# AIML-IfI/openset-imagenet

Measured on AMD Instinct MI355X. Metric: images/sec (whole node) ResNet-50 + entropic-open-set, Protocol 2, 1/2/4/8 GPUs, higher is better.
Workload: dtype f32; 1 GPU; Protocol 2, ResNet-50, entropic open-set loss, batch 128/GPU; workload_key=p2, classes=30, batch_per_gpu=128, global_batch=128, image=3x224x224, loss=entropic, optimizer=adam lr=1e-3, parallelism=dp1

## Files before the change

openset-imagenet_amd/csrc/conv_igemm.hip:

```cpp
#include "conv_common.h"
#include <algorithm>
#include <type_traits>

using namespace osi_conv;

namespace {

constexpr int BK = 32;
constexpr int LDR = BK + 4;

struct ConvP {
    const float* x;
    const float* w;
    float* y;
    int B, H, W, Cin, Ho, Wo, Cout, R, S, stride, pad;
    int M;
    int Ktot;
    int MT, NT;
    int accumulate;
    int x_bytes, w_bytes;
    FastDiv dHoWo, dWo;
    FastDiv cHW[4], cW[4];
    int unit;
    float* pmean;
// ... 826 lines not shown
#pragma unroll
        for (int i = 0; i < BRN; ++i) *reinterpret_cast<f32x4*>(sB + (bk_row + BRP * i) * LDC + bk_col) = rbv[i];
    };

    if (T > t0) {
        gload(); advance();
        sstore(0);
        __syncthreads();
        OSI_STAMP(p, sidx, 1);
            for (int t = t0; t < T; ++t) {
            const int buf = NST == 2 ? ((t - t0) & 1) : 0;
                if (!(OSI_ABLATE & 1)) if (t + 1 < T) { gload(); advance(); }
            const float* sA = smem + buf * STAGE;
            if (OSI_ABLATE & 16) {
#pragma unroll
                for (int j = 0; j < 16; ++j)
#pragma unroll
                    for (int i = 0; i < WM; ++i)
#pragma unroll
                        for (int n = 0; n < WN; ++n) acc[i][n] = __builtin_amdgcn_mfma_f32_32x32x2f32(ra[i % AR][j & 3], rbv[n % BRN][j & 3], acc[i][n], 0, 0, 0);
            } else if constexpr (W3) {
                const int h4 = (lane >> 5) * 4;
                const float* pa = sA + (prow + 2 - cjs) * LDR + h4;
                const float* pb = sA + AROWS * LDR + h4 * LDC + wn * 32 + (lane & 31);
#pragma unroll
                for (int j = 0; j < 4; ++j) {
                    const f32x4 a = *reinterpret_cast<const f32x4*>(pa + 8 * j);
#pragma unroll
                    for (int e = 0; e < 4; ++e) acc[0][0] = __builtin_amdgcn_mfma_f32_32x32x2f32(a[e], pb[(8 * j + e) * LDC], acc[0][0], 0, 0, 0);
                }
                if (++cjs == 3) cjs = 0;
            } else
            mma_RC<WM, WN, LDC>(sA, sA + BM * LDR, wm * 32 * WM, wn * 32 * WN, lane, acc);
            if (!(OSI_ABLATE & 4)) if (NST == 1) __syncthreads();
            if (!(OSI_ABLATE & 2)) if (t + 1 < T) sstore(NST == 2 ? (buf ^ 1) : 0);
            if (!(OSI_ABLATE & 4)) __syncthreads();
        }
        OSI_STAMP(p, sidx, 2);
    }
    if (OSI_ABLATE & 32) { if (acc[0][0][0] == 123.456f) p.y[tid] = acc[0][0][1]; return; }

    if constexpr (WM == 1 && WN == 1) {
        static_assert(BM * LDT <= STAGE, "transposed tile must fit the operand stage");
        float* tile = smem;
        tile64_to_lds<W3>(tile, acc[0][0], wm, wn, lane, m0, Mc);
        __syncthreads();
        if (KS && ks >= 0) {
            tile64_to_slab(p, tile, mt, nt, ks);
            OSI_STAMP(p, sidx, 3);
            return;
        }
        dgrad_epilogue64<FUSED, POOL>(p, smem, cls, mt, m0, n0, Mc, st, ph, pw, dHW, dW,
                                [&](int rl, int c4) { return *reinterpret_cast<const f32x4*>(tile + rl * LDT + c4 * 4); });
        OSI_STAMP(p, sidx, 3);
        return;
    }

    float esg[WN], es0[WN], es1[WN];
#pragma unroll
    for (int n = 0; n < WN; ++n) { esg[n] = 0.f; es0[n] = 0.f; es1[n] = 0.f; }
#pragma unroll
    for (int i = 0; i < WM; ++i) {
#pragma unroll
        for (int q = 0; q < 4; ++q) {
            uint32_t roff[4];
            bool rok[4];
#pragma unroll
            for (int e = 0; e < 4; ++e) {
                int m = m0 + wm * 32 * WM + i * 32 + acc_row(4 * q + e, lane);
                rok[e] = m < Mc;
                uint32_t mm = rok[e] ? (uint32_t)m : 0u;
                uint32_t pix;
                if (st == 1) pix = mm;
                else {
                    uint32_t b = fdiv(mm, dHW);
                    uint32_t rem = mm - b * dHW.d;
                    uint32_t h2 = fdiv(rem, dW), w2 = rem - h2 * dW.d;
                    pix = (b * p.H + (ph + st * h2)) * p.W + (pw + st * w2);
                }
                roff[e] = pix * p.Cin;
            }
#pragma unroll
            for (int n = 0; n < WN; ++n) {
                const int col = n0 + wn * 32 * WN + n * 32 + (lane & 31);
                float v[4];
#pragma unroll
                for (int e = 0; e < 4; ++e) v[e] = acc[i][n][4 * q + e];
                if (p.addend) {
#pragma unroll
                    for (int e = 0; e < 4; ++e) v[e] += rok[e] ? p.addend[roff[e] + col] : 0.f;
                }
                if (FUSED) {
                    if (p.ebits) {
#pragma unroll
                        for (int e = 0; e < 4; ++e) {
                            const uint32_t i4 = (roff[e] + col) >> 2;
                            const unsigned long long w = rok[e] ? p.ebits[(size_t)(i4 >> 6) * 4 + (col & 3)] : 0ull;
                            v[e] = (w >> (i4 & 63)) & 1 ? v[e] : 0.f;
                        }
                    }
                    if (p.escale0) {
                        const float gsc = p.escale0[col], gsh = p.eshift0[col];
#pragma unroll
                        for (int e = 0; e < 4; ++e)
                            v[e] = (rok[e] && __builtin_fmaf(p.ey0[roff[e] + col], gsc, gsh) > 0.f) ? v[e] : 0.f;
                    }
                    if (p.esum) {
                        const float mu0 = p.emean0[col], is0 = p.einv0[col];
#pragma unroll
                        for (int e = 0; e < 4; ++e) {
                            const float gv = rok[e] ? v[e] : 0.f;
                            esg[n] += gv;
                            es0[n] += gv * ((rok[e] ? p.ey0[roff[e] + col] : mu0) - mu0) * is0;
                        }
                        if (p.ey1) {
                            const float mu1 = p.emean1[col], is1 = p.einv1[col];
#pragma unroll
                            for (int e = 0; e < 4; ++e)
                                es1[n] += (rok[e] ? v[e] : 0.f) * ((rok[e] ? p.ey1[roff[e] + col] : mu1) - mu1) * is1;
                        }
                    }
                }
#pragma unroll
                for (int e = 0; e < 4; ++e)
                    if (rok[e]) p.y[roff[e] + col] = v[e];
            }
        }
    }
    if (FUSED && p.esum) {
#pragma unroll
        for (int n = 0; n < WN; ++n) {
            esg[n] += __shfl_xor(esg[n], 32, 64); es0[n] += __shfl_xor(es0[n], 32, 64); es1[n] += __shfl_xor(es1[n], 32, 64);
        }
        __syncthreads();
#pragma unroll
        for (int n = 0; n < WN; ++n)
            if (lane < 32) {
                float* dst = smem + (wm * BN + wn * 32 * WN + n * 32 + lane) * 3;
                dst[0] = esg[n]; dst[1] = es0[n]; dst[2] = es1[n];
            }
        __syncthreads();
        if (tid < BN) {
            const float* a = smem + tid * 3;
            const float* b = smem + (BN + tid) * 3;
            const size_t prow = (size_t)(cls * p.MT + mt) * p.Cin + n0 + tid;
            const size_t pstride = (size_t)p.eP * p.Cin;
            p.esum[prow] = a[0] + b[0];
            p.esum[pstride + prow] = a[1] + b[1];
            if (p.ey1) p.esum[2 * pstride + prow] = a[2] + b[2];
        }
    }
}

template <int WM, int WN, bool STEM, int NST, bool XF = false>
__global__ __launch_bounds__(256, NST == 1 ? (WM * WN == 4 ? 4 : (WM * WN == 2 ? 5 : 8)) : 2) void k_conv_wgrad(ConvP p) {
    static_assert(!(XF && STEM), "the stem reads the image, not an activation");
    constexpr int BM = 64 * WM, BN = 64 * WN;
    constexpr int LDA = BM + 4, LDB = BN + 4;
    constexpr int AV = BM / 4, ARP = 256 / AV, ARN = BK / ARP;
    constexpr int BV = BN / 4, BRP = 256 / BV, BRN = BK / BRP;
    constexpr int STAGE = BK * (LDA + LDB);
    extern __shared__ __attribute__((aligned(16))) float smem[];

    const int tid = threadIdx.x, lane = tid & 63, wave = tid >> 6;
    const int wm = wave >> 1, wn = wave & 1;
#ifdef OSI_STAMPS
    const size_t sidx = (size_t)blockIdx.y * gridDim.x + blockIdx.x;
#endif
    OSI_STAMP(p, sidx, 0); OSI_STAMP_ID(p, sidx);
    int mt, ntile, split;
    if (p.wgroup) {
        const int taps = STEM ? 1 : p.R * p.S;
        const int ctiles = p.NT / taps;
        const int xcd = blockIdx.x & 7, slot = blockIdx.x >> 3;
        const int u = slot % p.ginner;
        const int key = (slot / p.ginner) * 8 + xcd;
        if (key >= p.gkeys) return;
        const int tp = u % taps, v = u / taps;
        int ct;
        if (p.gkind == 0) { split = key; mt = v % p.MT; ct = v / p.MT; }
        else if (p.gkind == 1) { split = key / p.MT; mt = key - split * p.MT; ct = v; }
        else if (p.gkind == 2) { split = key / ctiles; ct = key - split * ctiles; mt = v; }
        else { mt = key % p.MT; const int rest = key / p.MT; ct = rest % ctiles; split = rest / ctiles; }
        ntile = tp * ctiles + ct;
    } else {
        mt = blockIdx.x % p.MT; ntile = blockIdx.x / p.MT; split = blockIdx.y;
    }
    const int n0 = mt * BM;
    int tap = 0, c0 = 0, r = 0, s = 0;
    if (!STEM) {
        const int ctiles = p.Cin / BN;
        tap = ntile / ctiles; c0 = (ntile - tap * ctiles) * BN;
        r = tap / p.S; s = tap - r * p.S;
    }
    const int kbeg = split * p.kchunk;
    const int kend = min(p.M, kbeg + p.kchunk);
    const int T = kend > kbeg ? (kend - kbeg + BK - 1) / BK : 0;

    f32x16 acc[WM][WN];
#pragma unroll
    for (int i = 0; i < WM; ++i)
#pragma unroll
        for (int n = 0; n < WN; ++n)
#pragma unroll
            for (int rr = 0; rr < 16; ++rr) acc[i][n][rr] = 0.f;

    const int a_row = tid / AV, a_col = (tid % AV) * 4;
    const int b_row = tid / BV, b_col = (tid % BV) * 4;
    f32x4 ra[ARN], rbv[BRN];

    const __amdgpu_buffer_rsrc_t rx = make_rsrc(p.x, p.x_bytes), rdy = make_rsrc(p.w, p.w_bytes);
    constexpr int TW = 32;
    uint32_t* tbl = reinterpret_cast<uint32_t*>(smem + NST * STAGE);
    const bool use_tbl = !STEM && p.wtbl;
    float* s_sc = smem + NST * STAGE + TW * BK;
    float* s_sh = s_sc + BN;
    if (XF) {
        if (tid < BN / 4) {
            *reinterpret_cast<f32x4*>(s_sc + tid * 4) = ld4(p.in_scale + c0 + tid * 4);
            *reinterpret_cast<f32x4*>(s_sh + tid * 4) = ld4(p.in_shift + c0 + tid * 4);
        }
        __syncthreads();
    }
    int ld_t = 0;
    auto build_tbl = [&](int t0) {
        for (int i = tid; i < TW * BK; i += 256) {
            const int m = kbeg + t0 * BK + i;
            uint32_t off = OOB;
            if (m < kend) {
                uint32_t b = fdiv((uint32_t)m, p.dHoWo);
                uint32_t rem = (uint32_t)m - b * p.dHoWo.d;
                uint32_t ho = fdiv(rem, p.dWo);
                uint32_t wo = rem - ho * p.dWo.d;
                int hi = (int)ho * p.stride - p.pad + r, wi = (int)wo * p.stride - p.pad + s;
                if ((unsigned)hi < (unsigned)p.H && (unsigned)wi < (unsigned)p.W)
                    off = (uint32_t)((((int)b * p.H + hi) * p.W + wi) * p.Cin * 4);
            }
            tbl[i] = off;
        }
        __syncthreads();
    };
    auto gload = [&](int t) {
        const int kb = kbeg + t * BK;
        ld_t = t;
#pragma unroll
        for (int i = 0; i < ARN; ++i) {
            const int m = kb + a_row + ARP * i;
            ra[i] = bld4(rdy, m < kend ? (uint32_t)(((a_row + ARP * i) * p.Cout + n0 + a_col) * 4) : OOB, (uint32_t)kb * p.Cout * 4);
        }
        if (!STEM) {
            uint32_t toff[BRN];
#pragma unroll
            for (int i = 0; i < BRN; ++i) toff[i] = tbl[(t % TW) * BK + b_row + BRP * i];
#pragma unroll
            for (int i = 0; i < BRN; ++i) {
                const int m = kb + b_row + BRP * i;
                const uint32_t uoff = m < kend ? (uint32_t)m * (uint32_t)(p.Cin * 4) : OOB;
                rbv[i] = bld4(rx, (p.unit ? uoff : toff[i]) + (uint32_t)((c0 + b_col) * 4), 0);
            }
        } else {
#pragma unroll
            for (int i = 0; i < BRN; ++i) {
                const int m = kb + b_row + BRP * i;
                bool ok = m < kend;
                uint32_t mm = ok ? (uint32_t)m : 0u;
                uint32_t b = fdiv(mm, p.dHoWo);
                uint32_t rem = mm - b * p.dHoWo.d;
                uint32_t ho = fdiv(rem, p.dWo);
                uint32_t wo = rem - ho * p.dWo.d;
                int rr = r, ss = s, coff = c0 + b_col;
                if (STEM) {
                    int tp = ntile * (BN / 4) + (b_col >> 2);
                    rr = tp / 7; ss = tp - rr * 7; coff = 0;
                    ok = ok && tp < 49;
                }
                int hi = (int)ho * p.stride - p.pad + rr, wi = (int)wo * p.stride - p.pad + ss;
                ok = ok && (unsigned)hi < (unsigned)p.H && (unsigned)wi < (unsigned)p.W;
                rbv[i] = bld4(rx, ok ? (uint32_t)(((((int)b * p.H + hi) * p.W + wi) * p.Cin + coff) * 4) : OOB, 0);
            }
        }
    };
    auto xform = [&]() {
        const f32x4 sc = *reinterpret_cast<const f32x4*>(s_sc + b_col), sh = *reinterpret_cast<const f32x4*>(s_sh + b_col);
#pragma unroll
        for (int i = 0; i < BRN; ++i) {
#pragma unroll
            for (int e = 0; e < 4; ++e) rbv[i][e] = osi_relu(__builtin_fmaf(rbv[i][e], sc[e], sh[e]));
        }
        if (!p.unit) {
#pragma unroll
            for (int i = 0; i < BRN; ++i) {
                const bool ok = tbl[(ld_t % TW) * BK + b_row + BRP * i] != OOB;
                rbv[i] = ok ? rbv[i] : f32x4{0.f, 0.f, 0.f, 0.f};
            }
        }
    };

    auto sstore = [&](int buf) {
        float* sA = smem + buf * STAGE;
        float* sB = sA + BK * LDA;
        if (XF) xform();
#pragma unroll
        for (int i = 0; i < ARN; ++i) *reinterpret_cast<f32x4*>(sA + (a_row + ARP * i) * LDA + a_col) = ra[i];
#pragma unroll
        for (int i = 0; i < BRN; ++i) *reinterpret_cast<f32x4*>(sB + (b_row + BRP * i) * LDB + b_col) = rbv[i];
    };
    if (T > 0) {
        if (use_tbl) build_tbl(0);
        gload(0);
        sstore(0);
        __syncthreads();
        OSI_STAMP(p, sidx, 1);
        for (int t = 0; t < T; ++t) {
            const int buf = NST == 2 ? (t & 1) : 0;
            if (use_tbl && t + 1 < T && (t + 1) % TW == 0) build_tbl(t + 1);
            if (!(OSI_ABLATE & 1)) if (t + 1 < T) gload(t + 1);
            const float* sA = smem + buf * STAGE;
            if (OSI_ABLATE & 16) {
#pragma unroll
                for (int ks = 0; ks < BK / 2; ++ks)
#pragma unroll
                    for (int i = 0; i < WM; ++i)
#pragma unroll
                        for (int n = 0; n < WN; ++n) acc[i][n] = __builtin_amdgcn_mfma_f32_32x32x2f32(ra[0][i & 3], rbv[0][n & 3], acc[i][n], 0, 0, 0);
            } else
            mma_CC<WM, WN, LDA, LDB>(sA, sA + BK * LDA, wm * 32 * WM, wn * 32 * WN, lane, acc);
            if (!(OSI_ABLATE & 4)) if (NST == 1) __syncthreads();
            if (!(OSI_ABLATE & 2)) if (t + 1 < T) sstore(NST == 2 ? (buf ^ 1) : 0);
            if (!(OSI_ABLATE & 4)) __syncthreads();
        }
        OSI_STAMP(p, sidx, 2);
    }

    float* out = p.y + (size_t)split * p.slab_stride;
    const int colbase = STEM ? ntile * BN : tap * p.Cin + c0;
#pragma unroll
    for (int i = 0; i < WM; ++i)
#pragma unroll
        for (int rr = 0; rr < 16; ++rr) {
            const int row = n0 + wm * 32 * WM + (WM == 2 ? 2 * acc_row(rr, lane) + i : acc_row(rr, lane));
            if constexpr (WN == 2) {
                const int col = colbase + wn * 64 + 2 * (lane & 31);
                if (col < p.Ktot) *reinterpret_cast<f32x2*>(out + (size_t)row * p.Ktot + col) = f32x2{acc[i][0][rr], acc[i][1][rr]};
            } else {
                const int col = colbase + wn * 32 + (lane & 31);
                if (col < p.Ktot) out[(size_t)row * p.Ktot + col] = acc[i][0][rr];
            }
        }
    OSI_STAMP(p, sidx, 3);
}

constexpr int W3_BKP = 32;
constexpr int W3_LDA = 64 + 16;
constexpr int W3_LDB = 32 + 16;
template <int NWIN, bool XF, bool S2 = false>
__global__ __launch_bounds__(256, 3) void k_conv_wgrad3(ConvP p) {
    extern __shared__ __attribute__((aligned(16))) float smem[];
    const int tid = threadIdx.x, lane = tid & 63, wave = tid >> 6;
    const int wn2 = wave >> 1, wc = wave & 1;
    OSI_STAMP(p, blockIdx.x, 0); OSI_STAMP_ID(p, blockIdx.x);
    const int W = p.W, WIN = S2 ? 130 + 2 * p.Wo : W3_BKP + 2 * W + 2;
    float* sA = smem;
    float* sB = sA + W3_BKP * W3_LDA;
    uint32_t* sM = reinterpret_cast<uint32_t*>(sB + NWIN * 32 * W3_LDB);
    const int ctiles = p.Cin / 32;
    int mt, ct, split;
    {
        const int xcd = blockIdx.x & 7, slot = blockIdx.x >> 3;
        const int u = slot % p.ginner, key = (slot / p.ginner) * 8 + xcd;
        if (key >= p.gkeys) return;
        if (p.gkind == 0) { split = key; mt = u % p.MT; ct = u / p.MT; }
        else { mt = key % p.MT; const int rest = key / p.MT; ct = rest % ctiles; split = rest / ctiles; }
    }
    const int n0 = mt * 64, c0 = ct * 32;
    const int kbeg = split * p.kchunk, kend = min(p.M, kbeg + p.kchunk);
    const int T = kend > kbeg ? (kend - kbeg + W3_BKP - 1) / W3_BKP : 0;

    f32x4acc acc[9][2];
#pragma unroll
    for (int t = 0; t < 9; ++t)
#pragma unroll
        for (int i = 0; i < 2; ++i) acc[t][i] = f32x4acc{0.f, 0.f, 0.f, 0.f};

    const __amdgpu_buffer_rsrc_t rx = make_rsrc(p.x, p.x_bytes), rdy = make_rsrc(p.w, p.w_bytes);
    const int a_row = tid >> 4, a_c4 = tid & 15;
    const int b_row = tid >> 3, b_c4 = tid & 7;
    f32x4 ra[2], rb[NWIN];
    f32x4 xsc = {0, 0, 0, 0}, xsh = xsc;
    if (XF) { xsc = ld4(p.in_scale + c0 + b_c4 * 4); xsh = ld4(p.in_shift + c0 + b_c4 * 4); }
    int s2_off[NWIN], s2_pq[NWIN], s2_c[NWIN];
    if (S2) {
        const int Wo = p.Wo;
#pragma unroll
        for (int i = 0; i < NWIN; ++i) {
            const int j = b_row + 32 * i;
            if (j < 32) { s2_pq[i] = 0; s2_off[i] = j; }
            else if (j < 65) { s2_pq[i] = 1; s2_off[i] = j - 32 - 1; }
            else if (j < 97 + Wo) { s2_pq[i] = 2; s2_off[i] = j - 65 - Wo; }
            else { s2_pq[i] = 3; s2_off[i] = j - (97 + Wo) - Wo - 1; }
            if (j >= WIN) s2_pq[i] = -1;
            s2_c[i] = (s2_pq[i] >> 1) * p.W + (s2_pq[i] & 1);
        }
    }

    auto gload = [&](int t) {
        const int q0 = kbeg + t * W3_BKP;
#pragma unroll
        for (int i = 0; i < 2; ++i) {
            const int q = q0 + a_row + 16 * i;
            ra[i] = bld4(rdy, q < kend ? (uint32_t)(((a_row + 16 * i) * p.Cout + n0 + a_c4 * 4) * 4) : OOB, (uint32_t)q0 * p.Cout * 4);
        }
        if constexpr (S2) {
#pragma unroll
            for (int i = 0; i < NWIN; ++i) {
                const int sq = q0 + s2_off[i];
                const bool in = s2_pq[i] >= 0 && sq >= 0 && sq < p.M;
                const uint32_t sqq = in ? (uint32_t)sq : 0u;
                const uint32_t wi = sqq - fdiv(sqq, p.dWo) * p.dWo.d;
                const uint32_t pix = 4 * sqq - 2 * wi + (uint32_t)s2_c[i];
                rb[i] = bld4(rx, in ? (pix * p.Cin + c0 + b_c4 * 4) * 4 : OOB, 0);
            }
        } else {
        const long wq0 = (long)q0 - W - 1;
#pragma unroll
        for (int i = 0; i < NWIN; ++i) {
            const int j = b_row + 32 * i;
            const long wq = wq0 + j;
            const bool in = j < WIN && wq >= 0 && wq < (long)p.M;
            rb[i] = bld4(rx, in ? (uint32_t)((wq * p.Cin + c0 + b_c4 * 4) * 4) : OOB, 0);
        }
        }
    };
    uint32_t mbits = 0;
    auto sstore = [&](int t) {
#pragma unroll
        for (int i = 0; i < 2; ++i) *reinterpret_cast<f32x4*>(sA + (a_row + 16 * i) * W3_LDA + a_c4 * 4) = ra[i];
#pragma unroll
        for (int i = 0; i < NWIN; ++i) *reinterpret_cast<f32x4*>(sB + (b_row + 32 * i) * W3_LDB + b_c4 * 4) = rb[i];
        if (tid < W3_BKP) sM[tid] = mbits;
    };
    auto xform = [&](int t) {
        if (XF) {
#pragma unroll
            for (int i = 0; i < NWIN; ++i)
#pragma unroll
                for (int e = 0; e < 4; ++e) rb[i][e] = osi_relu(__builtin_fmaf(rb[i][e], xsc[e], xsh[e]));
        }
        if (tid < W3_BKP) {
            const int q = kbeg + t * W3_BKP + tid;
            uint32_t bits = 0;
            if (q < kend) {
                const uint32_t b = fdiv((uint32_t)q, p.dHoWo);
                const uint32_t rem = (uint32_t)q - b * p.dHoWo.d;
                const int h = (int)fdiv(rem, p.dWo), w = (int)(rem - fdiv(rem, p.dWo) * p.dWo.d);
                const uint32_t rowm = (h > 0 ? 1u : 0u) | 2u | ((S2 || h < p.H - 1) ? 4u : 0u);
                const uint32_t colm = (w > 0 ? 1u : 0u) | 2u | ((S2 || w < p.W - 1) ? 4u : 0u);
#pragma unroll
                for (int r = 0; r < 3; ++r) if ((rowm >> r) & 1) bits |= colm << (3 * r);
            }
            mbits = bits;
        }
    };

    const int l15 = lane & 15, lk = lane >> 4;
    const int Wx = S2 ? p.Wo : W;
    const float* const bp0 = sB + lk * W3_LDB + 16 * wc + l15;
    const float* const bj[3] = {bp0, bp0 + Wx * W3_LDB, bp0 + 2 * Wx * W3_LDB};
    const float* const ap0 = sA + lk * W3_LDA + 32 * wn2 + l15;
    if (T > 0) {
        gload(0);
        xform(0);
        sstore(0);
        __syncthreads();
        OSI_STAMP(p, blockIdx.x, 1);
        for (int t = 0; t < T; ++t) {
            if (!(OSI_ABLATE & 1)) if (t + 1 < T) gload(t + 1);
            struct Ops { float a0, a1, b[9]; uint32_t m; };
            auto lds_ops = [&](int ks, Ops& o) {
                if (OSI_ABLATE & 16) {
                    o.a0 = __builtin_bit_cast(float, __builtin_bit_cast(uint32_t, o.a0) ^ (uint32_t)ks); return;
                }
                o.a0 = ap0[4 * ks * W3_LDA]; o.a1 = ap0[4 * ks * W3_LDA + 16];
                if (!(OSI_ABLATE & 8)) o.m = sM[4 * ks + lk];
#pragma unroll
                for (int tp = 0; tp < 9; ++tp) {
                    const int r = tp / 3, sx = tp % 3;
                    const int jb = !S2 ? r : (r == 2 ? 1 : 0) + (r != 1 && sx != 1 ? 1 : 0);
                    const int imm = !S2 ? sx : (r != 1 ? (sx != 1 ? 97 : 65) : (sx != 1 ? 32 : 0)) + (sx == 2 ? 1 : 0);
                    o.b[tp] = bj[jb][(4 * ks + imm) * W3_LDB];
                }
            };
            auto mma_ops = [&](const Ops& o) {
                const uint32_t mr0 = (uint32_t)((int)(o.m << 30) >> 31), mr2 = (uint32_t)((int)(o.m << 24) >> 31);
                const uint32_t ms0 = (uint32_t)((int)(o.m << 28) >> 31), ms2 = (uint32_t)((int)(o.m << 26) >> 31);
// ... 258 lines not shown
    int n = i / 224, k = i - n * 224, tap = k >> 2, c = k & 3;
    wp[i] = (tap < 49 && c < 3) ? w[(n * 49 + tap) * 3 + c] : 0.f;
}
__global__ void k_stem_unpack(const float* gp, float* g, int Cout) {
    int i = blockIdx.x * blockDim.x + threadIdx.x;
    if (i >= Cout * 147) return;
    int n = i / 147, k = i - n * 147, tap = k / 3, c = k - tap * 3;
    g[i] = gp[n * 224 + tap * 4 + c];
}

template <typename K>
static int set_smem(K kern, size_t bytes) {
    if (bytes > 64 * 1024) {
        if (hipFuncSetAttribute(reinterpret_cast<const void*>(kern), hipFuncAttributeMaxDynamicSharedMemorySize, (int)bytes) != hipSuccess)
            return OSI_ERR_LAUNCH;
    }
    return OSI_OK;
}

static bool desc_ok(const osi_conv_desc* d) {
    if (!d) return false;
    if (d->B <= 0 || d->H <= 0 || d->W <= 0 || d->Cin <= 0 || d->Cout <= 0) return false;
    if (d->R <= 0 || d->S <= 0 || d->stride <= 0 || d->pad < 0) return false;
    if (d->Ho != (d->H + 2 * d->pad - d->R) / d->stride + 1) return false;
    if (d->Wo != (d->W + 2 * d->pad - d->S) / d->stride + 1) return false;
    if (d->Ho <= 0 || d->Wo <= 0) return false;
    if ((long)d->B * d->H * d->W * d->Cin >= (1l << 29)) return false;
    if ((long)d->B * d->Ho * d->Wo * d->Cout >= (1l << 29)) return false;
    if ((long)d->Cout * d->R * d->S * (d->Cin < 4 ? 4 : d->Cin) >= (1l << 29)) return false;
    return true;
}
static bool is_stem(const osi_conv_desc* d) { return d->Cin == 4 && d->R == 7 && d->S == 7; }

enum ConvDir { DIR_FWD , DIR_DGRAD , DIR_WGRAD  };
static ConvP make_p(const osi_conv_desc* d, ConvDir dir) {
    ConvP p{};
    p.B = d->B; p.H = d->H; p.W = d->W; p.Cin = d->Cin; p.Ho = d->Ho; p.Wo = d->Wo; p.Cout = d->Cout;
    p.R = d->R; p.S = d->S; p.stride = d->stride; p.pad = d->pad;
    p.M = d->B * d->Ho * d->Wo;
    p.Ktot = is_stem(d) ? 224 : d->R * d->S * d->Cin;
    p.dHoWo = make_fastdiv((uint32_t)(d->Ho * d->Wo));
    p.dWo = make_fastdiv((uint32_t)d->Wo);
    p.unit = (d->R == 1 && d->S == 1 && d->stride == 1 && d->pad == 0) ? 1 : 0;
    const int in_bytes = (int)((size_t)d->B * d->H * d->W * d->Cin * 4), out_bytes = (int)((size_t)d->B * d->Ho * d->Wo * d->Cout * 4);
    p.x_bytes = dir == DIR_DGRAD ? out_bytes : in_bytes;
    p.w_bytes = dir == DIR_WGRAD ? out_bytes : (int)((size_t)d->Cout * p.Ktot * 4);
#ifdef OSI_STAMPS
    p.stamps = g_osi_stamps;
#endif
    return p;
}

struct TailPlan { int MT1, S, ksT, tiles; };
static TailPlan plan_tail_split(long MT, int NT, int T) {
    TailPlan t{(int)MT, 1, T, 0};
    if (!g_osi_tuning.tail_split || T < 4 || g_osi_tuning.tail_mint < 1) return t;
    const long ncu = chip_cus(), V = MT * NT;
    const long q = V / ncu, r = V - q * ncu;
    if (r == 0 || q > g_osi_tuning.tail_qmax) return t;
    if ((double)(ncu - r) / (double)ncu / (double)(q + 1) * 100.0 < (double)g_osi_tuning.tail_gain) return t;
    long MT1 = q * ncu / NT;
    long rem = (MT - MT1) * NT;
    long S = ncu / rem;
    if (S > T / g_osi_tuning.tail_mint) S = T / g_osi_tuning.tail_mint;
    if (S > g_osi_tuning.tail_smax) S = g_osi_tuning.tail_smax;
    if (q <= 2) {
        const long smax = std::min<long>(g_osi_tuning.tail_smax, T / g_osi_tuning.tail_mint);
        double best = S >= 2 ? 1.0 / (double)S : 1.0;
        for (long c = 2; c <= smax; ++c) {
            const double cost = (double)((rem * c + ncu - 1) / ncu) / (double)c;
            if (cost < best - 1e-9) { best = cost; S = c; }
        }
        if ((1.0 - best) / (double)(q + 1) * 100.0 < (double)g_osi_tuning.tail_gain) return t;
    }
    if (S <= 1) return t;
    const int ksT = (int)((T + S - 1) / S);
    S = (T + ksT - 1) / ksT;
    if (S <= 1) return t;
    t.MT1 = (int)MT1; t.S = (int)S; t.ksT = ksT; t.tiles = (int)rem;
    return t;
}
static size_t tail_slab_floats(const TailPlan& t) { return t.S > 1 ? (size_t)t.tiles * t.S * 4096 : 0; }

static int set_tail_split(ConvP& p, const TailPlan& tp, float* slab) {
    p.MT1 = tp.MT1; p.ks_S = tp.S; p.ks_T = tp.ksT; p.ks_slab = slab;
    p.g1 = osi_cdiv(p.MT1, 8) * 8 * p.NT;
    const int keys = (p.MT - p.MT1) * tp.S;
    return p.g1 + osi_cdiv(keys, 8) * 8 * p.NT;
}

template <int WM, int WN, bool STEM, int NST = 2, int XF = 0, bool W3 = false, bool OE = false, bool SPLIT = false>
static int launch_fwd(ConvP p, hipStream_t st, const TailPlan* tp = nullptr, float* slab = nullptr) {
    constexpr int BM = 64 * WM, BN = 64 * WN;
    p.MT = osi_cdiv(p.M, BM); p.NT = p.Cout / BN;
    size_t smem = NST * (size_t)((W3 ? W3_WROWS : BM) + BN) * LDR * sizeof(float);
    if (XF) smem += (size_t)2 * p.Cin * sizeof(float);
    if (W3) p.cW[0] = make_fastdiv((uint32_t)p.W + 1);
    if (int e = set_smem(k_conv_fwd<WM, WN, STEM, NST, XF, SPLIT, W3, OE>, smem)) return e;
    const int grid = SPLIT ? set_tail_split(p, *tp, slab) : osi_cdiv(p.MT, 8) * 8 * p.NT;
    hipLaunchKernelGGL((k_conv_fwd<WM, WN, STEM, NST, XF, SPLIT, W3, OE>), dim3(grid), dim3(256), smem, st, p);
    OSI_LAUNCH_CHECK();
    if constexpr (SPLIT) {
        hipLaunchKernelGGL(k_conv_fwd_tail_fixup, dim3(tp->tiles), dim3(256), 0, st, p);
        OSI_LAUNCH_CHECK();
    }
    return OSI_OK;
}
template <int KT, int XF, bool OE = false>
static int launch_fwd_rows(ConvP p, hipStream_t st) {
    p.MT = osi_cdiv(p.M, 64); p.NT = p.Cout / 64;
    int walkers = (4 * hw_cus() / p.NT + 7) / 8 * 8;
    if (walkers < 8) walkers = 8;
    if (walkers > p.MT) walkers = (p.MT + 7) / 8 * 8;
    const size_t smem = ((size_t)2 * KT * 64 * LDR + 2 * p.Cin + 2 * 64 * 3) * sizeof(float);
    if (int e = set_smem(k_conv1x1_rows<KT, XF, OE>, smem)) return e;
    hipLaunchKernelGGL((k_conv1x1_rows<KT, XF, OE>), dim3(walkers * p.NT), dim3(256), smem, st, p, walkers);
    OSI_LAUNCH_CHECK();
    return OSI_OK;
}
static bool rows_rule(const osi_conv_desc* d, bool shortcut) {
    const int m = g_osi_tuning.fwd_rows;
    const bool unit = d->R == 1 && d->S == 1 && d->stride == 1 && d->pad == 0;
    if (!m || !unit || shortcut || d->Cout % 64 || (d->Cin != 64 && d->Cin != 128)) return false;
    return m == 2 || (d->Cin == 64 && (long)d->B * d->Ho * d->Wo >= 64L * 8 * hw_cus());
}

template <int WM, int WN, int NST, int FUSED, bool POOL = false, bool W3 = false, bool SPLIT = false>
static int launch_dgrad(ConvP p, hipStream_t st, const TailPlan* tp = nullptr, float* slab = nullptr) {
    constexpr int BM = 64 * WM, BN = 64 * WN;
    const int s = p.stride;
    for (int ph = 0; ph < s; ++ph)
        for (int pw = 0; pw < s; ++pw) {
            const int hc = (p.H - ph + s - 1) / s, wc = (p.W - pw + s - 1) / s;
            p.cHW[ph * s + pw] = make_fastdiv((uint32_t)(hc * wc > 0 ? hc * wc : 1));
            p.cW[ph * s + pw] = make_fastdiv((uint32_t)(wc > 0 ? wc : 1));
        }
    p.unit = (p.R == 1 && p.S == 1 && s == 1 && p.pad == 0) ? 1 : 0;
    const int Hc = osi_cdiv(p.H, s), Wc = osi_cdiv(p.W, s);
    p.MT = osi_cdiv((long)p.B * Hc * Wc, BM); p.NT = p.Cin / BN;
    size_t smem = 2 * (size_t)((W3 ? W3_WROWS : BM) * LDR + BK * (BN + 4)) * sizeof(float);
    smem = smem / 2 * NST;
    if (W3) p.cW[1] = make_fastdiv((uint32_t)p.W + 1);
    if (int e = set_smem(k_conv_dgrad<WM, WN, NST, FUSED, SPLIT, POOL, W3>, smem)) return e;
    const int grid = SPLIT ? set_tail_split(p, *tp, slab) : osi_cdiv(p.MT, 8) * 8 * p.NT;
    hipLaunchKernelGGL((k_conv_dgrad<WM, WN, NST, FUSED, SPLIT, POOL, W3>), dim3(grid, s * s), dim3(256), smem, st, p, Hc, Wc);
    OSI_LAUNCH_CHECK();
    if constexpr (SPLIT) {
        hipLaunchKernelGGL(k_conv_dgrad_tail_fixup<FUSED>, dim3(tp->tiles), dim3(256), 0, st, p);
        OSI_LAUNCH_CHECK();
    }
    return OSI_OK;
}

template <int WM, int WN, bool STEM, int NST = 2, bool XF = false>
static int launch_wgrad(ConvP p, int splits, hipStream_t st) {
    constexpr int BM = 64 * WM, BN = 64 * WN;
    p.MT = p.Cout / BM;
    p.NT = STEM ? osi_cdiv(p.Ktot, BN) : p.R * p.S * (p.Cin / BN);
    size_t smem = 2 * (size_t)BK * (BM + 4 + BN + 4) * sizeof(float);
    smem = smem / 2 * NST;
    p.wtbl = (!STEM && !p.unit) ? 1 : 0;
    smem += 32 * BK * sizeof(uint32_t);
    if (XF) smem += 2 * BN * sizeof(float);
    if (int e = set_smem(k_conv_wgrad<WM, WN, STEM, NST, XF>, smem)) return e;
    p.splits = splits;
    p.wgroup = g_osi_tuning.wgrad_group;
    if (p.wgroup) {
        const int taps = STEM ? 1 : p.R * p.S;
        const int ctiles = p.NT / taps;
        if (p.wgroup == 1) { p.gkind = 3; p.gkeys = p.MT * ctiles * splits; p.ginner = taps; }
        else if (splits >= 8) { p.gkind = 0; p.gkeys = splits; p.ginner = p.MT * ctiles * taps; }
        else {
            const double dy_bytes = (double)p.Cout, x_bytes = (double)p.Cin;
            const double cost_rows = x_bytes * (p.MT < 8 ? p.MT : 8) + dy_bytes, cost_cols = dy_bytes * (ctiles < 8 ? ctiles : 8) + x_bytes;
            if (cost_rows <= cost_cols) { p.gkind = 1; p.gkeys = splits * p.MT; p.ginner = ctiles * taps; }
            else { p.gkind = 2; p.gkeys = splits * ctiles; p.ginner = p.MT * taps; }
        }
        const long grid = ((long)p.gkeys + 7) / 8 * 8 * p.ginner;
        hipLaunchKernelGGL((k_conv_wgrad<WM, WN, STEM, NST, XF>), dim3((unsigned)grid), dim3(256), smem, st, p);
    } else {
        hipLaunchKernelGGL((k_conv_wgrad<WM, WN, STEM, NST, XF>), dim3(p.MT * p.NT, splits), dim3(256), smem, st, p);
    }
    OSI_LAUNCH_CHECK();
    return OSI_OK;
}

static bool wgrad3_ok(const osi_conv_desc* d) {
    if (!g_osi_tuning.wgrad3 || d->R != 3 || d->S != 3 || d->pad != 1 || d->Cin % 32 || d->Cout % 64) return false;
    if (d->stride == 1) return d->W <= 63;
    return d->stride == 2 && g_osi_tuning.wgrad3 >= 2 && d->H % 2 == 0 && d->W % 2 == 0 && 130 + 2 * d->Wo <= 192;
}
template <int NWIN, bool XF, bool S2 = false>
static int launch_wgrad3_n(ConvP p, int splits, hipStream_t st) {
    p.MT = p.Cout / 64;
    const int ctiles = p.Cin / 32;
    p.splits = splits;
    if (splits >= 8) { p.gkind = 0; p.gkeys = splits; p.ginner = p.MT * ctiles; }
    else { p.gkind = 3; p.gkeys = p.MT * ctiles * splits; p.ginner = 1; }
    const size_t smem = ((size_t)W3_BKP * W3_LDA + (size_t)NWIN * 32 * W3_LDB + 32) * sizeof(float);
    if (int e = set_smem(k_conv_wgrad3<NWIN, XF, S2>, smem)) return e;
    const long grid = ((long)p.gkeys + 7) / 8 * 8 * p.ginner;
    hipLaunchKernelGGL((k_conv_wgrad3<NWIN, XF, S2>), dim3((unsigned)grid), dim3(256), smem, st, p);
    OSI_LAUNCH_CHECK();
    return OSI_OK;
}
template <bool XF>
static int launch_wgrad3(const ConvP& p, int splits, hipStream_t st) {
    if (p.stride == 2) return 130 + 2 * p.Wo <= 160 ? launch_wgrad3_n<5, XF, true>(p, splits, st) : launch_wgrad3_n<6, XF, true>(p, splits, st);
    const int win = W3_BKP + 2 * p.W + 2;
    if (win <= 64) return launch_wgrad3_n<2, XF>(p, splits, st);
    if (win <= 96) return launch_wgrad3_n<3, XF>(p, splits, st);
    return launch_wgrad3_n<5, XF>(p, splits, st);
}

struct TileShape { int wm, wn, nst; };
static TileShape tile_shape(int tile) {
    static const TileShape ids[9] = {{0, 0, 0}, {2, 2, 2}, {2, 1, 2}, {1, 2, 2}, {1, 1, 2}, {1, 1, 1}, {1, 2, 1}, {2, 2, 1}, {2, 1, 1}};
    return tile >= 1 && tile <= 8 ? ids[tile] : ids[0];
}
static int tile_rows(int tile) { return tile_shape(tile).wm == 2 ? 128 : 64; }
template <class F>
static int with_shape(TileShape s, F&& f) {
    return pick<1, 2>(s.wm, [&](auto WM) {
        return pick<1, 2>(s.wn, [&](auto WN) {
            return pick<1, 2>(s.nst, [&](auto NST) { return f(WM, WN, NST); });
        });
    });
}
enum LaunchForm { FORM_PLAIN = 0, FORM_POOL = 1, FORM_W3 = 2, FORM_SPLIT = 4 };

static bool row_window_shape(const osi_conv_desc* d) {
    return d->R == 3 && d->S == 3 && d->stride == 1 && d->pad == 1 && d->W >= 7 && d->H == d->Ho && d->W == d->Wo;
}

static size_t fwd_stats_floats(const osi_conv_desc* d) {
    const size_t n = bn_pstats_floats(osi_cdiv((long)d->B * d->Ho * d->Wo, 64), d->Cout);
    return (n + 63) / 64 * 64;
}
static TailPlan tail_plan(const osi_conv_desc* d, bool dgrad) {
    const long M = (long)d->B * (dgrad ? d->H * d->W : d->Ho * d->Wo);
    const int cols = dgrad ? d->Cin : d->Cout, kc = dgrad ? d->Cout : d->Cin;
    if (is_stem(d) || cols % 64 || kc % BK || (dgrad && d->stride != 1)) return TailPlan{(int)osi_cdiv(M, 64), 1, 0, 0};
    return plan_tail_split(osi_cdiv(M, 64), cols / 64, d->R * d->S * kc / BK);
}
enum FwdKind { FWD_STEM_DIRECT, FWD_STEM_GEMM, FWD_ROWS, FWD_SPLIT, FWD_W3, FWD_TILE };
struct FwdPlan {
    FwdKind kind;
    int tile;
    bool w3;
    TailPlan tail;
    int stat_rows;
    size_t slab_off;
};
static FwdPlan plan_fwd(const osi_conv_desc* d, int tile, bool shortcut, bool stats, size_t ws_bytes) {
    FwdPlan pl{FWD_TILE, tile, false, tail_plan(d, false), 64, stats ? fwd_stats_floats(d) : 0};
    if (is_stem(d)) {
        const bool direct = tile == OSI_TILE_AUTO && stem_direct_geometry(d);
        pl.kind = direct ? FWD_STEM_DIRECT : FWD_STEM_GEMM;
        pl.stat_rows = direct ? STEM_TILE_PIXELS : 128;
        return pl;
    }
    if (tile == OSI_TILE_AUTO) {
        if (rows_rule(d, shortcut)) { pl.kind = FWD_ROWS; return pl; }
        pl.w3 = g_osi_tuning.fwd_w3 && !shortcut && row_window_shape(d);
        const bool split = pl.tail.S > 1 && ws_bytes >= (pl.slab_off + tail_slab_floats(pl.tail)) * sizeof(float);
        if (split || pl.w3) { pl.kind = split ? FWD_SPLIT : FWD_W3; pl.tile = OSI_TILE_64x64_S1; return pl; }
        const long tiles64 = ((long)d->B * d->Ho * d->Wo + 63) / 64 * (d->Cout / 64);
        pl.tile = (tiles64 < 1024 && d->Cout % 128 == 0) ? OSI_TILE_64x128_S1 : OSI_TILE_64x64_S1;
        if (g_osi_tuning.fwd_wide && d->Cout % 128 == 0) pl.tile = OSI_TILE_64x128_S1;
    }
    pl.stat_rows = tile_rows(pl.tile);
    return pl;
}

constexpr bool fwd_kernel_exists(int wm, int wn, int nst, int xf, bool split, bool w3, bool oe) {
    if ((oe && xf != 0) || (w3 && xf == 2)) return false;
    if (split || w3) return wm == 1 && wn == 1 && nst == 1;
    return (xf == 0 && !oe) || (wm == 1 && nst == 1);
}
template <int XF, bool OE>
static int launch_fwd_plan(const FwdPlan& pl, const ConvP& p, float* ws, hipStream_t st) {
    if (pl.kind == FWD_STEM_GEMM) {
        if constexpr (XF == 0 && !OE) return launch_fwd<2, 1, true>(p, st);
        return OSI_ERR_ARG;
    }
    if (pl.kind == FWD_ROWS) {
        if constexpr (XF != 2) return p.Cin == 64 ? launch_fwd_rows<2, XF, OE>(p, st) : launch_fwd_rows<4, XF, OE>(p, st);
        return OSI_ERR_ARG;
    }
    auto go = [&](auto WM, auto WN, auto NST, auto FORM) -> int {
        constexpr int wm = decltype(WM)::value, wn = decltype(WN)::value, nst = decltype(NST)::value;
        constexpr bool w3 = (decltype(FORM)::value & FORM_W3) != 0, split = (decltype(FORM)::value & FORM_SPLIT) != 0;
        if constexpr (fwd_kernel_exists(wm, wn, nst, XF, split, w3, OE)) {
            if (wn == 2 && p.Cout % 128) return OSI_ERR_ARG;
            return launch_fwd<wm, wn, false, nst, XF, w3, OE, split>(p, st, &pl.tail, ws + pl.slab_off);
        } else return OSI_ERR_ARG;
    };
    const int form = (pl.w3 ? FORM_W3 : FORM_PLAIN) | (pl.kind == FWD_SPLIT ? FORM_SPLIT : FORM_PLAIN);
    return with_shape(tile_shape(pl.tile), [&](auto WM, auto WN, auto NST) {
        return pick<FORM_PLAIN, FORM_W3, FORM_SPLIT, FORM_W3 | FORM_SPLIT>(form, [&](auto FORM) { return go(WM, WN, NST, FORM); });
    });
}

static size_t dgrad_partial_floats(const osi_conv_desc* d) {
    const int s = d->stride;
    const long mt = osi_cdiv((long)d->B * osi_cdiv(d->H, s) * osi_cdiv(d->W, s), 64);
    return ((size_t)3 * s * s * mt * d->Cin + 63) / 64 * 64;
}
struct DgradPlan {
    int tile;
    int flavour;
    bool pool, w3, split;
    TailPlan tail;
    int P;
};
static DgradPlan plan_dgrad(const osi_conv_desc* d, int tile, const float* addend, const osi_dgrad_fusion* f, bool frozen) {
    DgradPlan pl{tile, 0, false, false, false, tail_plan(d, true), 0};
    const bool even_addend = f && f->addend_stride == 2;
    if (tile == OSI_TILE_AUTO) pl.tile = (g_osi_tuning.dgrad_wide && d->Cin % 128 == 0 && !even_addend) ? OSI_TILE_64x128_S1 : OSI_TILE_64x64_S1;
    const bool t64 = pl.tile == OSI_TILE_64x64_S1;
    if (frozen) pl.flavour = 4;
    else if (f && (f->relu_mask || f->partials || f->scale0)) {
        pl.pool = f->pool_idx != nullptr;
        if (pl.pool || tile_shape(pl.tile).wn == 2) pl.flavour = 1;
        else pl.flavour = (!addend && !f->relu_mask && !(f->partials && f->y1)) ? 2 : !f->scale0 ? 3 : 1;
    }
    pl.w3 = t64 && !pl.pool && (pl.flavour == 2 || pl.flavour == 4) && g_osi_tuning.dgrad_w3 && row_window_shape(d) && d->Cout % BK == 0 && d->Cin % 64 == 0;
    if (f && f->partials) {
        const int s = d->stride;
        pl.P = s * s * osi_cdiv((long)d->B * osi_cdiv(d->H, s) * osi_cdiv(d->W, s), tile_rows(pl.tile));
        pl.split = !pl.pool && t64 && pl.tail.S > 1 && f->partials_bytes >= (dgrad_partial_floats(d) + tail_slab_floats(pl.tail)) * sizeof(float);
    }
    return pl;
}
// ... 287 lines not shown
```

Measured before the change: 4516 images/sec.

## Run 128-wide wgrad tiles with eight waves per block

Adds an eight-wave (512-thread) variant of the weight-gradient implicit-GEMM kernel for non-stem 128x128 tiles, enabled by default, and optionally for 128x64 tiles via a build flag. Each wave now owns a smaller sub-tile of accumulators, so register pressure per wave drops and more waves can hide latency while staging the shared-memory tile with more loader threads. Load offsets are precomputed once, with the row offset moved into the buffer soffset. The cost is more synchronisation participants per barrier, a different launch-bounds occupancy target, and less MFMA reuse per wave.

```diff
diff --git a/openset-imagenet_amd/csrc/conv_igemm.hip b/openset-imagenet_amd/csrc/conv_igemm.hip
--- a/openset-imagenet_amd/csrc/conv_igemm.hip
+++ b/openset-imagenet_amd/csrc/conv_igemm.hip
@@ -1002,18 +1002,27 @@
     }
 }
 
-template <int WM, int WN, bool STEM, int NST, bool XF = false>
-__global__ __launch_bounds__(256, NST == 1 ? (WM * WN == 4 ? 4 : (WM * WN == 2 ? 5 : 8)) : 2) void k_conv_wgrad(ConvP p) {
+template <int NW, int WM, int WN, int NST>
+constexpr int wgrad_min_waves() {
+    if (NW == 8) return NST == 1 ? (WM * WN == 4 ? 7 : 8) : 4;
+    return NST == 1 ? (WM * WN == 4 ? 4 : (WM * WN == 2 ? 5 : 8)) : 2;
+}
+template <int WM, int WN, bool STEM, int NST, bool XF = false, int NW = 4>
+__global__ __launch_bounds__(64 * NW, (wgrad_min_waves<NW, WM, WN, NST>())) void k_conv_wgrad(ConvP p) {
     static_assert(!(XF && STEM), "the stem reads the image, not an activation");
+    static_assert(NW == 4 || (NW == 8 && !STEM && WM * WN >= 2), "eight waves: the 128-wide tiles only");
+    constexpr int NTH = 64 * NW;
+    constexpr int GM = NW == 8 ? 2 * WM : 2, GN = NW / GM;
+    constexpr int PM = 2 * WM / GM, PN = 2 * WN / GN;
     constexpr int BM = 64 * WM, BN = 64 * WN;
     constexpr int LDA = BM + 4, LDB = BN + 4;
-    constexpr int AV = BM / 4, ARP = 256 / AV, ARN = BK / ARP;
-    constexpr int BV = BN / 4, BRP = 256 / BV, BRN = BK / BRP;
+    constexpr int AV = BM / 4, ARP = NTH / AV, ARN = BK / ARP;
+    constexpr int BV = BN / 4, BRP = NTH / BV, BRN = BK / BRP;
     constexpr int STAGE = BK * (LDA + LDB);
     extern __shared__ __attribute__((aligned(16))) float smem[];
 
     const int tid = threadIdx.x, lane = tid & 63, wave = tid >> 6;
-    const int wm = wave >> 1, wn = wave & 1;
+    const int wm = wave / GN, wn = wave % GN;
 #ifdef OSI_STAMPS
     const size_t sidx = (size_t)blockIdx.y * gridDim.x + blockIdx.x;
 #endif
@@ -1047,16 +1056,17 @@
     const int kend = min(p.M, kbeg + p.kchunk);
     const int T = kend > kbeg ? (kend - kbeg + BK - 1) / BK : 0;
 
-    f32x16 acc[WM][WN];
-#pragma unroll
-    for (int i = 0; i < WM; ++i)
-#pragma unroll
-        for (int n = 0; n < WN; ++n)
+    f32x16 acc[PM][PN];
+#pragma unroll
+    for (int i = 0; i < PM; ++i)
+#pragma unroll
+        for (int n = 0; n < PN; ++n)
 #pragma unroll
             for (int rr = 0; rr < 16; ++rr) acc[i][n][rr] = 0.f;
 
     const int a_row = tid / AV, a_col = (tid % AV) * 4;
     const int b_row = tid / BV, b_col = (tid % BV) * 4;
+    const uint32_t a_off = (uint32_t)((a_row * p.Cout + n0 + a_col) * 4), b_off = (uint32_t)(b_row * p.Cin * 4);
     f32x4 ra[ARN], rbv[BRN];
 
     const __amdgpu_buffer_rsrc_t rx = make_rsrc(p.x, p.x_bytes), rdy = make_rsrc(p.w, p.w_bytes);
@@ -1074,7 +1084,7 @@
     }
     int ld_t = 0;
     auto build_tbl = [&](int t0) {
-        for (int i = tid; i < TW * BK; i += 256) {
+        for (int i = tid; i < TW * BK; i += NTH) {
             const int m = kbeg + t0 * BK + i;
             uint32_t off = OOB;
             if (m < kend) {
@@ -1096,7 +1106,10 @@
 #pragma unroll
         for (int i = 0; i < ARN; ++i) {
             const int m = kb + a_row + ARP * i;
-            ra[i] = bld4(rdy, m < kend ? (uint32_t)(((a_row + ARP * i) * p.Cout + n0 + a_col) * 4) : OOB, (uint32_t)kb * p.Cout * 4);
+            if constexpr (NW == 8)
+                ra[i] = bld4(rdy, tid < (kend - kb - ARP * i) * AV ? a_off : OOB, (uint32_t)(kb + ARP * i) * p.Cout * 4);
+            else
+                ra[i] = bld4(rdy, m < kend ? (uint32_t)(((a_row + ARP * i) * p.Cout + n0 + a_col) * 4) : OOB, (uint32_t)kb * p.Cout * 4);
         }
         if (!STEM) {
             uint32_t toff[BRN];
@@ -1105,8 +1118,14 @@
 #pragma unroll
             for (int i = 0; i < BRN; ++i) {
                 const int m = kb + b_row + BRP * i;
-                const uint32_t uoff = m < kend ? (uint32_t)m * (uint32_t)(p.Cin * 4) : OOB;
-                rbv[i] = bld4(rx, (p.unit ? uoff : toff[i]) + (uint32_t)((c0 + b_col) * 4), 0);
+                if constexpr (NW == 8) {
+                    const uint32_t uoff = tid < (kend - kb - BRP * i) * BV ? b_off : OOB;
+                    rbv[i] = bld4(rx, (p.unit ? uoff : toff[i]) + (uint32_t)((c0 + b_col) * 4),
+                                  p.unit ? (uint32_t)(kb + BRP * i) * (uint32_t)(p.Cin * 4) : 0u);
+                } else {
+                    const uint32_t uoff = m < kend ? (uint32_t)m * (uint32_t)(p.Cin * 4) : OOB;
+                    rbv[i] = bld4(rx, (p.unit ? uoff : toff[i]) + (uint32_t)((c0 + b_col) * 4), 0);
+                }
             }
         } else {
 #pragma unroll
@@ -1170,11 +1189,11 @@
 #pragma unroll
                 for (int ks = 0; ks < BK / 2; ++ks)
 #pragma unroll
-                    for (int i = 0; i < WM; ++i)
-#pragma unroll
-                        for (int n = 0; n < WN; ++n) acc[i][n] = __builtin_amdgcn_mfma_f32_32x32x2f32(ra[0][i & 3], rbv[0][n & 3], acc[i][n], 0, 0, 0);
+                    for (int i = 0; i < PM; ++i)
+#pragma unroll
+                        for (int n = 0; n < PN; ++n) acc[i][n] = __builtin_amdgcn_mfma_f32_32x32x2f32(ra[0][i & 3], rbv[0][n & 3], acc[i][n], 0, 0, 0);
             } else
-            mma_CC<WM, WN, LDA, LDB>(sA, sA + BK * LDA, wm * 32 * WM, wn * 32 * WN, lane, acc);
+            mma_CC<PM, PN, LDA, LDB>(sA, sA + BK * LDA, wm * 32 * PM, wn * 32 * PN, lane, acc);
             if (!(OSI_ABLATE & 4)) if (NST == 1) __syncthreads();
             if (!(OSI_ABLATE & 2)) if (t + 1 < T) sstore(NST == 2 ? (buf ^ 1) : 0);
             if (!(OSI_ABLATE & 4)) __syncthreads();
@@ -1185,11 +1204,11 @@
     float* out = p.y + (size_t)split * p.slab_stride;
     const int colbase = STEM ? ntile * BN : tap * p.Cin + c0;
 #pragma unroll
-    for (int i = 0; i < WM; ++i)
+    for (int i = 0; i < PM; ++i)
 #pragma unroll
         for (int rr = 0; rr < 16; ++rr) {
-            const int row = n0 + wm * 32 * WM + (WM == 2 ? 2 * acc_row(rr, lane) + i : acc_row(rr, lane));
-            if constexpr (WN == 2) {
+            const int row = n0 + wm * 32 * PM + (PM == 2 ? 2 * acc_row(rr, lane) + i : acc_row(rr, lane));
+            if constexpr (PN == 2) {
                 const int col = colbase + wn * 64 + 2 * (lane & 31);
                 if (col < p.Ktot) *reinterpret_cast<f32x2*>(out + (size_t)row * p.Ktot + col) = f32x2{acc[i][0][rr], acc[i][1][rr]};
             } else {
@@ -1754,9 +1773,16 @@
     return OSI_OK;
 }
 
+#ifndef OSI_WGRAD8
+#define OSI_WGRAD8 1
+#endif
+constexpr int wgrad_waves(int wm, int wn, bool stem) {
+    return !stem && ((wm * wn == 4 && (OSI_WGRAD8 & 1)) || (wm * wn == 2 && (OSI_WGRAD8 & 2))) ? 8 : 4;
+}
 template <int WM, int WN, bool STEM, int NST = 2, bool XF = false>
 static int launch_wgrad(ConvP p, int splits, hipStream_t st) {
-    constexpr int BM = 64 * WM, BN = 64 * WN;
+    constexpr int BM = 64 * WM, BN = 64 * WN, NW = wgrad_waves(WM, WN, STEM);
+    const auto kern = k_conv_wgrad<WM, WN, STEM, NST, XF, NW>;
     p.MT = p.Cout / BM;
     p.NT = STEM ? osi_cdiv(p.Ktot, BN) : p.R * p.S * (p.Cin / BN);
     size_t smem = 2 * (size_t)BK * (BM + 4 + BN + 4) * sizeof(float);
@@ -1764,7 +1790,7 @@
     p.wtbl = (!STEM && !p.unit) ? 1 : 0;
     smem += 32 * BK * sizeof(uint32_t);
     if (XF) smem += 2 * BN * sizeof(float);
-    if (int e = set_smem(k_conv_wgrad<WM, WN, STEM, NST, XF>, smem)) return e;
+    if (int e = set_smem(kern, smem)) return e;
     p.splits = splits;
     p.wgroup = g_osi_tuning.wgrad_group;
     if (p.wgroup) {
@@ -1779,9 +1805,9 @@
             else { p.gkind = 2; p.gkeys = splits * ctiles; p.ginner = p.MT * taps; }
         }
         const long grid = ((long)p.gkeys + 7) / 8 * 8 * p.ginner;
-        hipLaunchKernelGGL((k_conv_wgrad<WM, WN, STEM, NST, XF>), dim3((unsigned)grid), dim3(256), smem, st, p);
+        hipLaunchKernelGGL(kern, dim3((unsigned)grid), dim3(64 * NW), smem, st, p);
     } else {
-        hipLaunchKernelGGL((k_conv_wgrad<WM, WN, STEM, NST, XF>), dim3(p.MT * p.NT, splits), dim3(256), smem, st, p);
+        hipLaunchKernelGGL(kern, dim3(p.MT * p.NT, splits), dim3(64 * NW), smem, st, p);
     }
     OSI_LAUNCH_CHECK();
     return OSI_OK;
```

After: 4495 images/sec. About the same (-0.5%).
